# HuiGuanLab/Lite-MKD

Measured on AMD Instinct MI355X. Metric: episodes/sec (5-way 5-shot, 8x224^2 frames), higher is better.
Workload: dtype f32

## Files before the change

include/lmkd.h:

```cpp
#ifndef LMKD_H
#define LMKD_H
#ifdef __cplusplus
extern "C" {
#endif

int lmkd_abi_version(void);
const char* lmkd_last_error(void);
int lmkd_device_check(int device);
int lmkd_set_activation_dtype(int mode);
int lmkd_get_activation_dtype(void);

int lmkd_gemm_f32(char layA, char layB, int M, int N, int K, float alpha, const float* A, long lda, long sA,
                  const float* B, long ldb, long sB, float beta, float* C, long ldc, long sC, const float* bias,
                  int relu, int batch, void* stream);
int lmkd_gemm_set_mode(int mode);
int lmkd_gemm_set_tile(int t);
long lmkd_gemm_ticket_words(void);
int lmkd_gemm_f32_splitk(char layA, char layB, int M, int N, int K, float alpha, const float* A, long lda, long sA,
                         const float* B, long ldb, long sB, float beta, float* C, long ldc, long sC, const float* bias,
                         int relu, int batch, void* workspace, long ws_bytes, unsigned* tickets, void* stream);

long lmkd_conv2d_packed_weight_elems(int Cout, int Cin, int Cs, int KH, int KW, int mode);
int lmkd_conv2d_pack_weights(const float* w_oihw, float* wp, int Cout, int Cin, int Cs, int KH, int KW, int mode ,
                             void* stream);
int lmkd_conv2d_fwd_row_tiles(int N, int H, int W, int Cout, int KH, int KW, int stride, int pad);
int lmkd_conv2d_fwd_row_tiles_cs(int N, int H, int W, int Cs, int Cout, int KH, int KW, int stride, int pad);
int lmkd_set_elementwise_wg_per_cu(int n);
int lmkd_conv_set_compute_dtype(int mode);
typedef struct lmkd_amax_desc {
  const void* x_words;
  const void* dy_words;
  void* out_words;
  const void* ref_words;
  int flags;
} lmkd_amax_desc;
#define LMKD_AMAX_FENCED 1
int lmkd_h2_fence_eval(const void* const* words, void* const* refs, int n, int* flags, void* stream);
long lmkd_conv_h2_fallbacks(void);
int lmkd_amax(const float* x, long n, void* word, void* stream);
long lmkd_amax_words(void);
long lmkd_conv2d_plane_elems(int ncols, int Kp);
long lmkd_conv_h2_launches(void);
int lmkd_conv2d_repack_multi(const float* const* ws, void* const* wfs, const int* dims, int n, void* stream);
int lmkd_conv2d_split_weights(const float* wp, void* wf, int ncols, int Kp, void* stream);
int lmkd_conv_get_compute_dtype(void);
int lmkd_conv_set_wgrad_planes(int on);
int lmkd_conv_set_patch(int on);
int lmkd_conv_set_stem_patch(int on);
int lmkd_conv_set_s2_patch(int on);
int lmkd_conv_set_wgrad_win16(int on);
int lmkd_conv_set_wgrad_stem(int on);
int lmkd_conv_set_wgrad_window(int on);
int lmkd_conv_set_patch16(int on);
int lmkd_conv_set_persistent(int on);
int lmkd_conv_set_xcd_mode(int mode);
int lmkd_conv_set_tile(int id);
int lmkd_conv2d_fwd(const float* x, const float* wp_fwd, float* y, float* stat_partial, int N, int H, int W, int Cs, int Cout,
                    int KH, int KW, int stride, int pad, void* stream);
int lmkd_conv2d_fwd_pre(const float* x_raw, const float* pre_stats, const float* wp_fwd, float* y, float* stat_partial, int N, int H,
                        int W, int Cs, int Cout, int KH, int KW, int stride, int pad, void* stream);
int lmkd_conv2d_fwd_bn(const float* x, const float* wp_fwd, float* y, const float* bn_stats, const float* res , int relu,
                       int N, int H, int W, int Cs, int Cout, int KH, int KW, int stride, int pad, void* stream,
                       const lmkd_amax_desc* amax );
int lmkd_conv2d_bwd_data(const float* dy, const float* wp_dgrad, float* dx, int N, int H, int W, int Cin, int Cout, int KH, int KW,
                         int stride, int pad, int accumulate, void* stream);
int lmkd_conv2d_bwd_data_bn_tiles(int N, int H, int W, int Cin, int Cout, int KH, int KW, int stride, int pad);
int lmkd_conv2d_bwd_data_bn(const float* dy, const float* wp_dgrad, float* dx, const float* bn_x, const float* bn_stats, float* part,
                            int N, int H, int W, int Cin, int Cout, int KH, int KW, int stride, int pad, void* stream);
long lmkd_conv2d_bwd_weight_workspace(int N, int H, int W, int Cs, int Cout, int KH, int KW, int stride, int pad);
int lmkd_conv2d_bwd_weight(const float* x, const float* dy, float* dw_oihw, float* workspace, long ws_bytes, int N, int H, int W,
                           int Cs, int Cin, int Cout, int KH, int KW, int stride, int pad, void* stream);
int lmkd_conv2d_bwd_weight_pre(const float* x_raw, const float* pre_stats, const float* dy, float* dw_oihw, float* workspace,
                               long ws_bytes, int N, int H, int W, int Cs, int Cin, int Cout, int KH, int KW, int stride, int pad,
                               void* stream);

int lmkd_conv2d_plan(int kind, int N, int H, int W, int Cs, int Cin, int Cout, int KH, int KW, int stride, int pad, int* info_host);

int lmkd_conv2d_bwd_weight_acc(const float* x, const float* pre_stats, const float* dy, float* dw_oihw, float* workspace, long ws_bytes,
                               int N, int H, int W, int Cs, int Cin, int Cout, int KH, int KW, int stride, int pad, void* stream);

int lmkd_frames_u8_to_nhwc4(const unsigned char* src, float* dst, const int* crop_y, const int* crop_x, const int* flip, int F, int Hs,
                            int Ws, int H, int W, int frames_per_video, void* stream);
int lmkd_resize_plan(int in_size, int out_size, int* bounds_host, int* coeffs_host);
int lmkd_resize_pass_u8(const unsigned char* src, unsigned char* dst, const int* bounds_dev, const int* coeffs_dev, int ksize, long outer,
                        int n_in, int n_out, long inner, void* stream);
int lmkd_frames_resize_crop_nhwc4(const unsigned char* src, float* dst, const int* bounds_h, const int* coeffs_h, int ksize_h,
                                  const int* bounds_v, const int* coeffs_v, int ksize_v, const int* crop_y, const int* crop_x,
                                  const int* flip, int F, int Hs, int Ws, int Hr, int Wr, int H, int W, int frames_per_video, void* stream);
int lmkd_nchw3_to_nhwc4(const float* x_nchw, float* y_nhwc4, int N, int H, int W, void* stream, void* amax_words);
long lmkd_ticket_words(void);
int lmkd_bn_finalize(const float* partial, int T, int C, long count, const float* gamma, const float* beta, float* running_mean,
                     float* running_var, float momentum, float eps, float* stats, double* scratch, unsigned* tickets, void* stream,
                     const lmkd_amax_desc* amax );
int lmkd_bn_running_update(float* running_mean, float* running_var, const float* stats, int C, float momentum, void* stream);
int lmkd_bn_running_update_multi(float* const* running_mean, float* const* running_var, const float* const* stats_first,
                                 const float* const* stats_second, const int* C, int n, float momentum, void* stream);
int lmkd_bn_running_update_multi_nbt(float* const* running_mean, float* const* running_var, const float* const* stats_first,
                                     const float* const* stats_second, long long* const* num_batches_tracked, const int* C, int n,
                                     float momentum, void* stream);
int lmkd_bn_eval_stats(int C, const float* gamma, const float* beta, const float* running_mean, const float* running_var, float eps,
                       float* stats, void* stream);
int lmkd_bn_apply(const float* x, const float* stats, const float* res, const float* rstats, float* y, long rows, int C, int relu,
                  int res_mode, unsigned* mask_bits, void* stream);
long lmkd_bn_bwd_workspace(int C);
int lmkd_bn_backward(const float* dy, const float* x, const float* yact, const float* stats, const float* gamma, float* dx,
                     float* g_out, float* dgamma, float* dbeta, float* coef, void* workspace, unsigned* tickets, long rows, int C,
                     int mask_mode, int accumulate_param_grads, void* stream);
int lmkd_bn_backward_part(const float* part, int T, const float* dy, const float* x, const float* stats, const float* gamma, float* dx,
                          float* dgamma, float* dbeta, float* coef, void* workspace, unsigned* tickets, long rows, int C,
                          int accumulate_param_grads, void* stream);
int lmkd_relu_backward(const float* dy, const float* y, float* g, long n, void* stream);
int lmkd_bn_relu_maxpool_fwd(const float* x, const float* stats, float* y, unsigned char* idx, float* cmax, int N, int H, int W, int C,
                             void* stream);
int lmkd_maxpool_bwd(const float* dy, const unsigned char* idx, float* g, int N, int H, int W, int C, void* stream);
int lmkd_bn_backward_stats(const float* dy, const float* cmax, const float* stats, const float* gamma, float* dgamma, float* dbeta,
                           float* coef, void* workspace, unsigned* tickets, long pooled_rows, long count, int C, int accumulate_param_grads,
                           void* stream);
int lmkd_stem_unpool_bn_bwd(const float* dy, const unsigned char* idx, const float* c, const float* stats, const float* coef, float* dc,
                            int N, int H, int W, int C, void* stream, const lmkd_amax_desc* amax );
int lmkd_adaptive_maxpool_mean_fwd(const float* x, float* y, int F, int H, int W, int C, void* stream);
int lmkd_adaptive_maxpool_mean_bwd(const float* x, const float* dy, float* dx, int F, int H, int W, int C, void* stream);
long lmkd_colsum_workspace(int C);
int lmkd_colsum(const float* a, const float* b, float* out, long rows, int C, int accumulate, void* workspace, unsigned* tickets,
                void* stream);

int lmkd_dropout_mask(float* mask, long n, float p, unsigned long long seed, void* stream);
int lmkd_dropout_mask_dev(float* mask, long n, float p, const unsigned long long* seed_dev, void* stream);
int lmkd_add_pe(const float* x, const float* pe, const float* mask, float* y, long rows, int D, int L, void* stream);
int lmkd_mul(const float* a, const float* b, float* out, long n, void* stream);
int lmkd_axpby(const float* x, float* y, float alpha, float beta, long n, void* stream);
int lmkd_trx_tuple_ln_fwd(const float* P, const float* bk, const float* bv, const float* gamma, const float* beta, const int* rowmap,
                          float* Kn, float* Khat, float* V, float* rstd, int NV, int L, int D, float eps, void* stream);
int lmkd_layernorm_bwd_rows(float* dK_inout, const float* Khat, const float* rstd, const float* gamma, long rows, int D, void* stream);
int lmkd_trx_tuple_bwd_gather(const float* dKraw, const float* dV, const int* rowmap, float* dP, int NV, int L, int D, void* stream);
int lmkd_segment_softmax_fwd(float* S, long rows, long ld, int nseg, const int* seg_off, const int* seg_cnt, void* stream);
int lmkd_segment_softmax_bwd(const float* P, float* dP_inout, long rows, long ld, int nseg, const int* seg_off, const int* seg_cnt,
                             void* stream);
// ... 68 lines not shown
```

lite-mkd_amd/_lib.py:

```python
import ctypes
import os
import re

from . import _audit

_HERE = os.path.dirname(os.path.abspath(__file__))
_ROOT = os.path.dirname(_HERE)
HEADER = os.path.join(_ROOT, "include", "lmkd.h")
LIB_PATH = os.environ.get("LMKD_LIB") or os.path.join(_HERE, "liblmkd_hip.so")

_CT = {
    "int": ctypes.c_int, "long": ctypes.c_long, "float": ctypes.c_float, "char": ctypes.c_char,
    "long long": ctypes.c_longlong, "unsigned long long": ctypes.c_ulonglong,
}


def parse_header(path=HEADER):
    txt = open(path).read()
    txt = re.sub(r"/\*.*?\*/", " ", txt, flags=re.S)
    protos = {}
    for m in re.finditer(r"\b(int|long|const char\s*\*)\s+(lmkd_\w+)\s*\(([^)]*)\)\s*;", txt):
        ret, name, args = m.group(1), m.group(2), m.group(3).strip()
        restype = ctypes.c_char_p if "char" in ret else _CT[ret]
        argtypes = []
        if args and args != "void":
            for a in args.split(","):
                a = a.strip()
                if "*" in a:
                    argtypes.append(ctypes.c_void_p)
                else:
                    toks = a.replace("const ", "").split()
                    ty = " ".join(toks[:-1])
                    argtypes.append(_CT[ty])
        protos[name] = (restype, argtypes)
    return protos


class _Lib:
    def __init__(self):
        if not os.path.exists(LIB_PATH):
            raise RuntimeError(
                "liblmkd_hip.so not found at %s: build it with `python lite-mkd_amd/build.py` "
                "(there is no CPU or PyTorch fallback for the hot path)" % LIB_PATH)
        import torch
        self.cdll = ctypes.CDLL(LIB_PATH)
        self.protos = parse_header()
        for name, (restype, argtypes) in self.protos.items():
            fn = getattr(self.cdll, name)
            fn.restype = restype
            fn.argtypes = argtypes
        if os.environ.get("LMKD_PATCH16"):
            self.cdll.lmkd_conv_set_patch16(int(os.environ["LMKD_PATCH16"]))
        if os.environ.get("LMKD_WGRAD_WINDOW"):
            self.cdll.lmkd_conv_set_wgrad_window(int(os.environ["LMKD_WGRAD_WINDOW"]))
        if os.environ.get("LMKD_CONV_PERSISTENT", "1") == "0":
            self.cdll.lmkd_conv_set_persistent(0)

    def last_error(self):
        return self.cdll.lmkd_last_error().decode()

    def call(self, name, *args):
        if _audit.ON:
            _audit.check(name)
        rc = getattr(self.cdll, name)(*args)
        if rc != 0:
            raise RuntimeError("%s failed (%d): %s" % (name, rc, self.last_error()))

    def value(self, name, *args):
        return getattr(self.cdll, name)(*args)


_lib = None


def lib():
    global _lib
    if _lib is None:
        _lib = _Lib()
    return _lib
```

lite-mkd_amd/csrc/conv.hip:

```cpp
#include "gemm_core.h"
#include <atomic>
#include <mutex>

struct ConvGemmArgs {
  const float* src;
  const float* wpk;
  float* out;
  float* stat_partial;
  int N, Hs, Ws, Cs;
  int Hr, Wr, rows_per_class, tiles_per_class;
  int sh;
  int Ho, Wo, Co, omul;
  int Kp, cps, nclass;
  int n_rt, n_ct, xcd_mode;
  int taps_pm1;
  int grid_step;
  int grid_total;
  int same;
  int halo;
  int accum;
  const float* ep_stats;
  const float* ep_res;
  int ep_relu;
  const float* pre_stats;
// ... 784 lines not shown
template <class Cfg, bool SMALLC, int STATS, bool BF16 = false>
static void launch_conv_cfg(ConvGemmArgs a, int ncols, hipStream_t s) {
  conv_set_tiles(a, Cfg::BM);
  a.n_ct = cdiv(ncols, Cfg::BN);
  a.xcd_mode = (a.n_ct >= 8 && (a.n_ct & 7) == 0) ? 1 : 0;
  if (g_xcd_mode == 0) a.xcd_mode = 0;
  const dim3 grid(xcd_grid(a.n_rt, a.n_ct, a.xcd_mode));
  if constexpr (STATS == 1 && !SMALLC && !BF16) {
    if (a.pre_stats) {
      hipLaunchKernelGGL((conv_gemm_kernel<Cfg, SMALLC, STATS, BF16, true>), grid, dim3(Cfg::THREADS), 0, s, a);
      return;
    }
  }
  hipLaunchKernelGGL((conv_gemm_kernel<Cfg, SMALLC, STATS, BF16>), grid, dim3(Cfg::THREADS), 0, s, a);
}

static inline void lmkd_lds_attr_once(std::atomic<unsigned long long>& mask, const void* fn, int bytes) {
  int d = 0;
  if (hipGetDevice(&d) != hipSuccess) d = 0;
  const unsigned long long bit = 1ull << (d & 63);
  if (mask.load(std::memory_order_acquire) & bit) return;
  const hipError_t err = hipFuncSetAttribute(fn, hipFuncAttributeMaxDynamicSharedMemorySize, bytes);
  if (err != hipSuccess) {
    lmkd_set_error("hipFuncSetAttribute(MaxDynamicSharedMemorySize = %d): %s", bytes, hipGetErrorString(err));
    return;
  }
  mask.fetch_or(bit, std::memory_order_release);
}

struct PersistOcc { std::atomic<int> n{0}; int lds[8]; int occ[8]; std::mutex mu; };
static int lmkd_cu_count() {
  static std::atomic<int> n{0};
  int v = n.load(std::memory_order_relaxed);
  if (v) return v;
  int d = 0;
  hipDeviceProp_t pr;
  if (hipGetDevice(&d) != hipSuccess || hipGetDeviceProperties(&pr, d) != hipSuccess || pr.multiProcessorCount < 1) return 256;
  n.store(pr.multiProcessorCount, std::memory_order_relaxed);
  return pr.multiProcessorCount;
}
static int g_conv_persist = 1;
extern "C" int lmkd_conv_set_persistent(int on) { g_conv_persist = on ? 1 : 0; return LMKD_OK; }
template <class K>
static int persistent_grid(PersistOcc& c, K kernel, int threads, size_t lds, int total) {
  if (!g_conv_persist) return total;
  int occ = 0;
  {
    std::lock_guard<std::mutex> lk(c.mu);
    const int n = c.n.load();
    for (int i = 0; i < n; ++i) if (c.lds[i] == (int)lds) occ = c.occ[i];
    if (!occ) {
      if (hipOccupancyMaxActiveBlocksPerMultiprocessor(&occ, kernel, threads, lds) != hipSuccess || occ < 1) occ = 1;
      if (n < 8) { c.lds[n] = (int)lds; c.occ[n] = occ; c.n.store(n + 1); }
    }
  }
  const int slots = occ * lmkd_cu_count();
  if (total <= slots) return total;
  const int rounds = cdiv(total, slots);
  const int g = (cdiv(total, rounds) + 7) & ~7;
  return g < total ? g : total;
}

static int patch_halo(const ConvGemmArgs& a) {
  if (!g_conv_patch || !(g_conv_x3 || g_conv_bf16) || a.Cs % 32 != 0 || a.sh != 1) return -1;
  const bool plain = a.nclass == 1 && a.Hs == a.Ho && a.Ws == a.Wo;
  const bool classes = a.nclass == 4 && a.Hr == a.Hs && a.Wr == a.Ws;
  if (!plain && !classes) return -1;
  int halo = 0;
  for (int c = 0; c < a.nclass; ++c)
    for (int t = 0; t < a.ntap[c]; ++t) {
      const int sft = a.taps[c][t].dh * a.Ws + a.taps[c][t].dw;
      halo = std::max(halo, sft < 0 ? -sft : sft);
    }
  return halo <= PATCH_HALO_MAX ? halo : -1;
}
static inline bool conv_same_size(int H, int W, int KH, int KW, int stride, int pad) {
  return g_conv_patch && stride == 1 && conv_out(H, KH, stride, pad) == H && conv_out(W, KW, stride, pad) == W && (KH / 2) * W + KW / 2 <= PATCH_HALO_MAX;
}

static int g_conv_s2_patch = 1;
extern "C" int lmkd_conv_set_s2_patch(int on) { g_conv_s2_patch = on ? 1 : 0; return LMKD_OK; }
static int g_patch16 = 1;
extern "C" int lmkd_conv_set_patch16(int on) { g_patch16 = on < 0 ? 0 : (on > 2 ? 2 : on); return LMKD_OK; }

#ifdef LMKD_STAMPS
extern "C" int lmkd_debug_stamps(unsigned long long* host, int zero) {
  if (zero) {
    void* p = nullptr;
    if (hipGetSymbolAddress(&p, HIP_SYMBOL(g_lmkd_stamps)) != hipSuccess) return LMKD_EHIP;
    return hipMemset(p, 0, sizeof(g_lmkd_stamps)) == hipSuccess ? LMKD_OK : LMKD_EHIP;
  }
  return hipMemcpyFromSymbol(host, HIP_SYMBOL(g_lmkd_stamps), sizeof(g_lmkd_stamps)) == hipSuccess ? LMKD_OK : LMKD_EHIP;
}
#endif
static inline int taps_within_one(const ConvGemmArgs& a) {
  for (int c = 0; c < a.nclass; ++c)
    for (int t = 0; t < a.ntap[c]; ++t)
      if (a.taps[c][t].dh < -1 || a.taps[c][t].dh > 1 || a.taps[c][t].dw < -1 || a.taps[c][t].dw > 1) return 0;
  return 1;
}
template <class Cfg>
static void launch_conv_patch(ConvGemmArgs a, int ncols, int halo, hipStream_t s) {
  conv_set_tiles(a, Cfg::BM);
  a.taps_pm1 = taps_within_one(a);
  a.n_ct = cdiv(ncols, Cfg::BN);
  a.xcd_mode = (a.n_ct >= 8 && (a.n_ct & 7) == 0) ? 1 : 0;
  if (g_xcd_mode == 0) a.xcd_mode = 0;
  const dim3 grid(xcd_grid(a.n_rt, a.n_ct, a.xcd_mode));
  a.halo = halo;
  const int npl = (g_conv_bf16 || g_lmkd_act_bf16) ? 1 : 3;
  size_t lds = patch_lds_bytes(Cfg::BM, halo, npl);
#define LMKD_PATCH(NPROD, PRE, IO)                                                                                             \
  do {                                                                                                                         \
    static std::atomic<unsigned long long> attr_done{0};                                                                       \
    static PersistOcc pocc;                                                                                                    \
    lmkd_lds_attr_once(attr_done, reinterpret_cast<const void*>(&conv_patch_x3_kernel<Cfg, NPROD, PRE, IO>),                   \
                       (int)patch_lds_bytes(Cfg::BM, PATCH_HALO_MAX, NPROD == 1 ? 1 : 3));                                     \
    a.grid_total = (int)grid.x;                                                                                                \
    const dim3 pgrid(NPROD == 3 ? persistent_grid(pocc, conv_patch_x3_kernel<Cfg, NPROD, PRE, IO>, Cfg::THREADS, lds, a.grid_total) : a.grid_total); \
    a.grid_step = (int)pgrid.x;                                                                                                \
    hipLaunchKernelGGL((conv_patch_x3_kernel<Cfg, NPROD, PRE, IO>), pgrid, dim3(Cfg::THREADS), lds, s, a);                     \
  } while (0)
  if constexpr (Cfg::THREADS == 256 && Cfg::BM == 128) {
    const bool h2_on_32 = g_patch16 == 1 && Cfg::BN == 64 && a.Co <= 64 && g_conv_h2 && a.h2_xw && !a.src2 && !a.ep_stats;
    if (g_patch16 && g_conv_x3 && !g_lmkd_act_bf16 && !h2_on_32) {
#define LMKD_PATCH16(NPROD, PRE, EP)                                                                                           \
  do {                                                                                                                         \
    t_amax_recorded = true;                                                                                                    \
    static std::atomic<unsigned long long> attr_done{0};                                                                       \
    lmkd_lds_attr_once(attr_done, reinterpret_cast<const void*>(&conv_patch16_x3_kernel<Cfg, NPROD, PRE, EP>),                 \
                       (int)patch_lds_bytes(Cfg::BM, PATCH_HALO_MAX, 3));                                                      \
    hipLaunchKernelGGL((conv_patch16_x3_kernel<Cfg, NPROD, PRE, EP>), grid, dim3(Cfg::THREADS), lds, s, a);                    \
  } while (0)
      if (a.src2) {
#define LMKD_PATCH16S(NPROD, EP)                                                                                               \
  do {                                                                                                                         \
    t_amax_recorded = true;                                                                                                    \
    static std::atomic<unsigned long long> attr_done{0};                                                                       \
    lmkd_lds_attr_once(attr_done, reinterpret_cast<const void*>(&conv_patch16_x3_kernel<Cfg, NPROD, false, EP, true>),         \
                       (int)patch_lds_bytes(Cfg::BM, PATCH_HALO_MAX, 3));                                                      \
    hipLaunchKernelGGL((conv_patch16_x3_kernel<Cfg, NPROD, false, EP, true>), grid, dim3(Cfg::THREADS), lds, s, a);            \
  } while (0)
        if (a.ep_stats) {
          if (g_conv_x3 == 9) LMKD_PATCH16S(9, true);
          else if (g_conv_h2 && a.h2_xw) { LMKD_PATCH16S(3, true); ++g_h2_launches; }
          else LMKD_PATCH16S(6, true);
        }
        else if (g_conv_h2 && a.h2_xw) { LMKD_PATCH16S(3, false); ++g_h2_launches; }
        else { if (g_conv_x3 == 9) LMKD_PATCH16S(9, false); else LMKD_PATCH16S(6, false); }
#undef LMKD_PATCH16S
        return;
      }
      if (a.ep_stats) {
        if (g_conv_x3 == 9) LMKD_PATCH16(9, false, true);
        else if (g_conv_h2 && a.h2_xw) { LMKD_PATCH16(3, false, true); ++g_h2_launches; }
        else LMKD_PATCH16(6, false, true);
      }
      else if (a.pre_stats) {
        if (g_conv_x3 == 9) LMKD_PATCH16(9, true, false);
        else if (g_conv_h2 && a.h2_xw) { LMKD_PATCH16(3, true, false); ++g_h2_launches; }
        else LMKD_PATCH16(6, true, false);
      }
      else if (a.bnb_x) {
#define LMKD_PATCH16B(NPROD)                                                                                                   \
  do {                                                                                                                         \
    t_amax_recorded = true;                                                                                                    \
    static std::atomic<unsigned long long> attr_done{0};                                                                       \
    lmkd_lds_attr_once(attr_done, reinterpret_cast<const void*>(&conv_patch16_x3_kernel<Cfg, NPROD, false, false, false, true>), \
                       (int)patch_lds_bytes(Cfg::BM, PATCH_HALO_MAX, 3));                                                      \
    hipLaunchKernelGGL((conv_patch16_x3_kernel<Cfg, NPROD, false, false, false, true>), grid, dim3(Cfg::THREADS), lds, s, a);  \
  } while (0)
        if (g_conv_h2 && a.h2_xw) { LMKD_PATCH16B(3); ++g_h2_launches; }
        else if (g_conv_x3 == 9) LMKD_PATCH16B(9);
        else LMKD_PATCH16B(6);
#undef LMKD_PATCH16B
      }
      else if (g_conv_h2 && a.h2_xw) { LMKD_PATCH16(3, false, false); ++g_h2_launches; }
      else { if (g_conv_x3 == 9) LMKD_PATCH16(9, false, false); else LMKD_PATCH16(6, false, false); }
#undef LMKD_PATCH16
      return;
    }
  }
  if (g_conv_h2 && a.h2_xw && !a.ep_stats && !g_lmkd_act_bf16) {
    t_amax_recorded = true;
    lds = patch_lds_bytes(Cfg::BM, halo, 2);
    if (a.pre_stats) LMKD_PATCH(3, true, 0); else LMKD_PATCH(3, false, 0);
    ++g_h2_launches;
    return;
  }
  if (a.ep_stats) {
    if (g_conv_bf16) LMKD_PATCH(1, false, 4);
    else if (g_conv_x3 == 9) LMKD_PATCH(9, false, 4);
    else LMKD_PATCH(6, false, 4);
  } else if (g_lmkd_act_bf16) LMKD_PATCH(1, false, 3);
  else if (a.pre_stats) {
    if (g_conv_bf16) LMKD_PATCH(1, true, 0);
    else if (g_conv_x3 == 9) LMKD_PATCH(9, true, 0);
    else LMKD_PATCH(6, true, 0);
  } else {
    if (g_conv_bf16) LMKD_PATCH(1, false, 0);
    else if (g_conv_x3 == 9) LMKD_PATCH(9, false, 0);
    else LMKD_PATCH(6, false, 0);
  }
#undef LMKD_PATCH
}

template <class Cfg>
static void launch_conv_patch_1p(ConvGemmArgs a, int ncols, int halo, hipStream_t s) {
  conv_set_tiles(a, Cfg::BM);
  a.taps_pm1 = taps_within_one(a);
  a.n_ct = cdiv(ncols, Cfg::BN);
  a.xcd_mode = (a.n_ct >= 8 && (a.n_ct & 7) == 0) ? 1 : 0;
  if (g_xcd_mode == 0) a.xcd_mode = 0;
  const dim3 grid(xcd_grid(a.n_rt, a.n_ct, a.xcd_mode));
  a.halo = halo;
  const size_t lds = patch_lds_bytes(Cfg::BM, halo, 1);
#define LMKD_PATCH1(PRE, IO)                                                                                                   \
  do {                                                                                                                         \
    static std::atomic<unsigned long long> attr_done{0};                                                                       \
    lmkd_lds_attr_once(attr_done, reinterpret_cast<const void*>(&conv_patch_x3_kernel<Cfg, 1, PRE, IO>),                       \
                       (int)patch_lds_bytes(Cfg::BM, PATCH_HALO_MAX, 1));                                                      \
    a.grid_total = (int)grid.x;                                                                                                \
    const dim3 pgrid(a.grid_total);                  \
    a.grid_step = (int)pgrid.x;                                                                                                \
    hipLaunchKernelGGL((conv_patch_x3_kernel<Cfg, 1, PRE, IO>), pgrid, dim3(Cfg::THREADS), lds, s, a);                         \
  } while (0)
  if (a.ep_stats) LMKD_PATCH1(false, 4);
  else if (g_lmkd_act_bf16) LMKD_PATCH1(false, 3);
  else if (a.pre_stats) LMKD_PATCH1(true, 0);
  else LMKD_PATCH1(false, 0);
#undef LMKD_PATCH1
}

template <class Cfg, bool SMALLC, bool STATS>
static void launch_conv_x3(ConvGemmArgs a, int ncols, hipStream_t s) {
  conv_set_tiles(a, Cfg::BM);
  a.n_ct = cdiv(ncols, Cfg::BN);
  a.xcd_mode = (a.n_ct >= 8 && (a.n_ct & 7) == 0) ? 1 : 0;
  if (g_xcd_mode == 0) a.xcd_mode = 0;
  const dim3 grid(xcd_grid(a.n_rt, a.n_ct, a.xcd_mode));
  (void)STATS;
  if constexpr (!SMALLC) {
    if (a.ep_stats) {
      if (g_conv_bf16) hipLaunchKernelGGL((conv_gemm_x3_kernel<Cfg, false, true, 1, false, 4>), grid, dim3(Cfg::THREADS), 0, s, a);
      else if (g_conv_x3 == 9) hipLaunchKernelGGL((conv_gemm_x3_kernel<Cfg, false, true, 9, false, 4>), grid, dim3(Cfg::THREADS), 0, s, a);
      else hipLaunchKernelGGL((conv_gemm_x3_kernel<Cfg, false, true, 6, false, 4>), grid, dim3(Cfg::THREADS), 0, s, a);
      return;
    }
  }
  if (g_lmkd_act_bf16) {
    if constexpr (SMALLC) hipLaunchKernelGGL((conv_gemm_x3_kernel<Cfg, true, true, 1, false, 2>), grid, dim3(Cfg::THREADS), 0, s, a);
    else hipLaunchKernelGGL((conv_gemm_x3_kernel<Cfg, false, true, 1, false, 3>), grid, dim3(Cfg::THREADS), 0, s, a);
    return;
  }
  if constexpr (!SMALLC) {
    if (a.pre_stats) {
      if (g_conv_bf16) hipLaunchKernelGGL((conv_gemm_x3_kernel<Cfg, false, true, 1, true>), grid, dim3(Cfg::THREADS), 0, s, a);
      else if (g_conv_x3 == 9) hipLaunchKernelGGL((conv_gemm_x3_kernel<Cfg, false, true, 9, true>), grid, dim3(Cfg::THREADS), 0, s, a);
      else hipLaunchKernelGGL((conv_gemm_x3_kernel<Cfg, false, true, 6, true>), grid, dim3(Cfg::THREADS), 0, s, a);
      return;
    }
  }
  if (g_conv_bf16) hipLaunchKernelGGL((conv_gemm_x3_kernel<Cfg, SMALLC, true, 1>), grid, dim3(Cfg::THREADS), 0, s, a);
  else if (g_conv_x3 == 9) hipLaunchKernelGGL((conv_gemm_x3_kernel<Cfg, SMALLC, true, 9>), grid, dim3(Cfg::THREADS), 0, s, a);
  else hipLaunchKernelGGL((conv_gemm_x3_kernel<Cfg, SMALLC, true, 6>), grid, dim3(Cfg::THREADS), 0, s, a);
}

template <bool SMALLC, int STATS>
// ... 720 lines not shown
```

lite-mkd_amd/csrc/conv_patch.h:

```cpp
#pragma once

#define PATCH_HALO_MAX 57

template <int NPL> struct PatchRow { static constexpr int BYTES = NPL == 1 ? 80 : (NPL == 2 ? 144 : 208); };

static inline size_t patch_lds_bytes(int bm, int halo, int npl) { return (size_t)(bm + 2 * halo + 1) * (npl == 1 ? 80 : (npl == 2 ? 144 : 208)); }

#ifdef LMKD_STAMPS
__device__ unsigned long long g_lmkd_stamps[4096 * 8];
#define STAMP(k) do { if (threadIdx.x == 0 && (blockIdx.x & 63) == 0 && (blockIdx.x >> 6) < 4096) g_lmkd_stamps[(blockIdx.x >> 6) * 8 + (k)] = __builtin_amdgcn_s_memtime(); } while (0)
#else
#define STAMP(k) do { } while (0)
#endif


template <class Cfg>
__device__ __forceinline__ void patch_h2_epilogue(const ConvGemmArgs& a, f32x16 (&acc)[Cfg::TM][Cfg::TN], const int* s_out, float* s_red, int rt,
                                                  int n0, int wm, int wn, int lane, int tid, int seg, int row0, int M, float h2_ix, float h2_iw) {
  const int cl0 = wn * (Cfg::TN * 32) + (lane & 31);
  const bool bnb = a.bnb_x != nullptr;
  float s1[Cfg::TN], s2[Cfg::TN];
  float amo = 0.f;
  const bool plain = a.nclass == 1;
  const int rows = M - row0 < Cfg::BM ? M - row0 : Cfg::BM;
// ... 411 lines not shown
      read_a(0);
      if (AHEAD) read_a(1);
      __builtin_amdgcn_sched_barrier(0);
#pragma unroll
      for (int g = 0; g < 2; ++g) {
        const int ga = AHEAD ? g : 0;
        if (!AHEAD && g == 1) {
          __builtin_amdgcn_sched_barrier(0);
          read_a(1);
          __builtin_amdgcn_sched_barrier(0);
        }
#pragma unroll
        for (int j = 0; j < Cfg::TN; ++j) {
          if constexpr (NPROD == 1) {
            const bf16x8 b0 = x3_as_bf16(rb[j * 2 + g]);
#pragma unroll
            for (int i = 0; i < Cfg::TM; ++i) acc[i][j] = __builtin_amdgcn_mfma_f32_32x32x16_bf16(av[ga][0][i], b0, acc[i][j], 0, 0, 0);
          } else if constexpr (NPROD == 3) {
            const f16x8 b0 = __builtin_bit_cast(f16x8, rb[j * 4 + g * 2 + 0]), b1 = __builtin_bit_cast(f16x8, rb[j * 4 + g * 2 + 1]);
#pragma unroll
            for (int i = 0; i < Cfg::TM; ++i) {
              f32x16 c = acc[i][j];
              c = __builtin_amdgcn_mfma_f32_32x32x16_f16(__builtin_bit_cast(f16x8, av[ga][0][i]), b1, c, 0, 0, 0);
              c = __builtin_amdgcn_mfma_f32_32x32x16_f16(__builtin_bit_cast(f16x8, av[ga][1][i]), b0, c, 0, 0, 0);
              c = __builtin_amdgcn_mfma_f32_32x32x16_f16(__builtin_bit_cast(f16x8, av[ga][0][i]), b0, c, 0, 0, 0);
              acc[i][j] = c;
            }
          } else {
            const bf16x8 b0 = x3_as_bf16(rb[j * 6 + g * 3 + 0]), b1 = x3_as_bf16(rb[j * 6 + g * 3 + 1]), b2 = x3_as_bf16(rb[j * 6 + g * 3 + 2]);
#pragma unroll
            for (int i = 0; i < Cfg::TM; ++i) {
              f32x16 c = acc[i][j];
              if (NPROD == 9) {
                c = __builtin_amdgcn_mfma_f32_32x32x16_bf16(av[ga][2][i], b2, c, 0, 0, 0);
                c = __builtin_amdgcn_mfma_f32_32x32x16_bf16(av[ga][1][i], b2, c, 0, 0, 0);
                c = __builtin_amdgcn_mfma_f32_32x32x16_bf16(av[ga][2][i], b1, c, 0, 0, 0);
              }
              c = __builtin_amdgcn_mfma_f32_32x32x16_bf16(av[ga][1][i], b1, c, 0, 0, 0);
              c = __builtin_amdgcn_mfma_f32_32x32x16_bf16(av[ga][0][i], b2, c, 0, 0, 0);
              c = __builtin_amdgcn_mfma_f32_32x32x16_bf16(av[ga][2][i], b0, c, 0, 0, 0);
              c = __builtin_amdgcn_mfma_f32_32x32x16_bf16(av[ga][0][i], b1, c, 0, 0, 0);
              c = __builtin_amdgcn_mfma_f32_32x32x16_bf16(av[ga][1][i], b0, c, 0, 0, 0);
              c = __builtin_amdgcn_mfma_f32_32x32x16_bf16(av[ga][0][i], b0, c, 0, 0, 0);
              acc[i][j] = c;
            }
          }
        }
      }
      if (++k_tp == ntap) { k_tp = 0; ++k_cc; }
      __builtin_amdgcn_sched_barrier(0);
      x3_landed(rbn);
      x3_landed(rp);
      __builtin_amdgcn_sched_barrier(0);
      if (t + 2 < nk) issue_b(rb);
    };
    PSTAMP(1);
    if (nk > 0) {
      x3_landed(rp);
      x3_landed(rb0);
      x3_landed(rb1);
      __builtin_amdgcn_sched_barrier(0);
      PSTAMP(2);
      int t = 0;
      for (; t + 1 < nk; t += 2) {
        step(t, rb0, rb1, avp0, avp1);
        step(t + 1, rb1, rb0, avp1, avp0);
      }
      if (t < nk) step(t, rb0, rb1, avp0, avp1);
    }
    PSTAMP(3);
    if constexpr (NPROD == 3) {
      patch_h2_epilogue<Cfg>(a, acc, s_out, s_red, cur.rt, n0, wm, wn, lane, tid, cur.seg, row0, M, h2_ix, h2_iw);
    } else {
      x3_epilogue<Cfg, true, OUT16, EP>(a, acc, s_out, s_red, cur.rt, n0, wm, wn, lane, tid, neg);
    }
    PSTAMP(4);
    if (!PERSIST || Ln < 0) break;
    if (!inv) __syncthreads();
    cur = nxt;
    Lc = Ln;
    ++it;
  }
}
```

Before: 51.32.

## Add ring-buffered persistent patch kernel for 64-channel 3x3 split-half conv

Adds a persistent conv kernel for the 64-channel 3x3 stride-1 two-plane (h2) case. It keeps a rolling LDS ring of input pixel rows so consecutive output tiles handled by one block reuse the overlapping halo instead of reloading it, and it prefetches the next tile's new rows while the current tile's MFMAs run. The aim is to cut redundant global loads and halo staging per tile. In exchange it adds a specialised code path with strict eligibility conditions, more LDS use, and a fixed row-ordering assumption about ring slots.

```diff
diff --git a/include/lmkd.h b/include/lmkd.h
--- a/include/lmkd.h
+++ b/include/lmkd.h
@@ -53,6 +53,7 @@
 int lmkd_conv_set_wgrad_window(int on);
 int lmkd_conv_set_patch16(int on);
 int lmkd_conv_set_persistent(int on);
+int lmkd_conv_set_patch_ring(int on);
 int lmkd_conv_set_xcd_mode(int mode);
 int lmkd_conv_set_tile(int id);
 int lmkd_conv2d_fwd(const float* x, const float* wp_fwd, float* y, float* stat_partial, int N, int H, int W, int Cs, int Cout,
diff --git a/lite-mkd_amd/_lib.py b/lite-mkd_amd/_lib.py
--- a/lite-mkd_amd/_lib.py
+++ b/lite-mkd_amd/_lib.py
@@ -55,6 +55,8 @@
             self.cdll.lmkd_conv_set_wgrad_window(int(os.environ["LMKD_WGRAD_WINDOW"]))
         if os.environ.get("LMKD_CONV_PERSISTENT", "1") == "0":
             self.cdll.lmkd_conv_set_persistent(0)
+        if os.environ.get("LMKD_CONV_PATCH_RING", "1") == "0":
+            self.cdll.lmkd_conv_set_patch_ring(0)
 
     def last_error(self):
         return self.cdll.lmkd_last_error().decode()
diff --git a/lite-mkd_amd/csrc/conv.hip b/lite-mkd_amd/csrc/conv.hip
--- a/lite-mkd_amd/csrc/conv.hip
+++ b/lite-mkd_amd/csrc/conv.hip
@@ -890,6 +890,12 @@
 extern "C" int lmkd_conv_set_s2_patch(int on) { g_conv_s2_patch = on ? 1 : 0; return LMKD_OK; }
 static int g_patch16 = 1;
 extern "C" int lmkd_conv_set_patch16(int on) { g_patch16 = on < 0 ? 0 : (on > 2 ? 2 : on); return LMKD_OK; }
+static int g_patch_ring = 1;
+extern "C" int lmkd_conv_set_patch_ring(int on) { g_patch_ring = on ? 1 : 0; return LMKD_OK; }
+static inline bool patch_ring_fits(const ConvGemmArgs& a, int halo) {
+  return g_patch_ring && g_conv_persist && a.nclass == 1 && a.n_ct == 1 && !a.src2 && a.Cs == 64 && a.cps == 2 && a.ntap[0] == 9 && a.taps_pm1 &&
+         halo <= 64 && a.n_rt > 0;
+}
 
 #ifdef LMKD_STAMPS
 extern "C" int lmkd_debug_stamps(unsigned long long* host, int zero) {
@@ -992,6 +998,24 @@
   if (g_conv_h2 && a.h2_xw && !a.ep_stats && !g_lmkd_act_bf16) {
     t_amax_recorded = true;
     lds = patch_lds_bytes(Cfg::BM, halo, 2);
+    if constexpr (Cfg::BM == 128 && Cfg::BN == 64 && Cfg::THREADS == 256 && Cfg::TN == 1) {
+      if (patch_ring_fits(a, halo)) {
+        const size_t rlds = patch_ring_lds_bytes();
+#define LMKD_PATCH_RING(PRE)                                                                                                   \
+  do {                                                                                                                         \
+    static std::atomic<unsigned long long> attr_done{0};                                                                       \
+    static PersistOcc pocc;                                                                                                    \
+    lmkd_lds_attr_once(attr_done, reinterpret_cast<const void*>(&conv_patch_ring_kernel<Cfg, PRE>), (int)rlds);               \
+    a.grid_total = a.n_rt;                                                                                                     \
+    a.grid_step = persistent_grid(pocc, conv_patch_ring_kernel<Cfg, PRE>, Cfg::THREADS, rlds, a.n_rt);                         \
+    hipLaunchKernelGGL((conv_patch_ring_kernel<Cfg, PRE>), dim3(a.grid_step), dim3(Cfg::THREADS), rlds, s, a);                 \
+  } while (0)
+        if (a.pre_stats) LMKD_PATCH_RING(true); else LMKD_PATCH_RING(false);
+#undef LMKD_PATCH_RING
+        ++g_h2_launches;
+        return;
+      }
+    }
     if (a.pre_stats) LMKD_PATCH(3, true, 0); else LMKD_PATCH(3, false, 0);
     ++g_h2_launches;
     return;
diff --git a/lite-mkd_amd/csrc/conv_patch.h b/lite-mkd_amd/csrc/conv_patch.h
--- a/lite-mkd_amd/csrc/conv_patch.h
+++ b/lite-mkd_amd/csrc/conv_patch.h
@@ -517,3 +517,208 @@
     ++it;
   }
 }
+
+#define RING_ROWB 272
+#define RING_ROWS 256
+static inline size_t patch_ring_lds_bytes() { return (size_t)(RING_ROWS + 1) * RING_ROWB; }
+
+template <class Cfg, bool PRE>
+__global__ __launch_bounds__(Cfg::THREADS, 2) void conv_patch_ring_kernel(ConvGemmArgs) {
+  static_assert(Cfg::BM == 128 && Cfg::THREADS == 256 && Cfg::BN == 64 && Cfg::TN == 1, "layer 1's two-plane tile");
+  __shared__ ConvGemmArgs s_args;
+  {
+    const unsigned* ksrc = (const unsigned*)__builtin_amdgcn_kernarg_segment_ptr();
+    unsigned* kdst = reinterpret_cast<unsigned*>(&s_args);
+    for (int i = threadIdx.x; i < (int)(sizeof(ConvGemmArgs) / 4); i += Cfg::THREADS) kdst[i] = ksrc[i];
+  }
+  __syncthreads();
+  ConvGemmArgs a;
+  {
+    constexpr int NW = (int)(offsetof(ConvGemmArgs, ntap) / 4);
+    unsigned* aw = reinterpret_cast<unsigned*>(&a);
+    const unsigned* lw = reinterpret_cast<const unsigned*>(&s_args);
+#pragma unroll
+    for (int i = 0; i < NW; ++i) aw[i] = __builtin_amdgcn_readfirstlane(lw[i]);
+  }
+  constexpr int ROWB = RING_ROWB, NTAP = 9, NK = 2 * NTAP;
+  constexpr int LPR = 16, RPP = Cfg::THREADS / LPR, NI = Cfg::BM / RPP;
+  using LB = X3FragB<Cfg::TN, 2>;
+  extern __shared__ __attribute__((aligned(16))) unsigned char psm[];
+  __shared__ unsigned short s_mask_lut[64];
+  __shared__ float s_red[Cfg::WM * Cfg::BN * 2];
+  const int tid = threadIdx.x;
+  const int lane = tid & 63, wave = tid >> 6;
+  const int wm = wave / Cfg::WN, wn = wave % Cfg::WN;
+  const int h = lane >> 5;
+  const int a_row = wm * (Cfg::TM * 32) + (lane & 31);
+  const unsigned zero_addr = (unsigned)(RING_ROWS * ROWB + 16 * h);
+  const __amdgpu_buffer_rsrc_t prs = x3_rsrc(a.src, (long)a.N * a.Hs * a.Ws * a.Cs * 4);
+  const int pk = (tid & (LPR - 1)) * 4;
+  const long src_pixels = (long)a.N * a.Hs * a.Ws;
+  const int G = a.grid_step, T = a.n_rt, b = (int)blockIdx.x;
+  const int r = (G & 7) == 0 ? (b & 7) * (G >> 3) + (b >> 3) : b;
+  const int t_beg = (int)((long)r * T / G), t_end = (int)((long)(r + 1) * T / G);
+  if (t_beg >= t_end) return;
+  const Tap my_tap = s_args.taps[0][lane < NTAP ? lane : 0];
+  int sh_px[NTAP], kofs[NTAP];
+#pragma unroll
+  for (int tp = 0; tp < NTAP; ++tp) {
+    sh_px[tp] = __builtin_amdgcn_readlane(my_tap.dh * a.Ws + my_tap.dw, tp);
+    kofs[tp] = __builtin_amdgcn_readlane(my_tap.kofs, tp);
+  }
+  if (tid < 64) {
+    const int rb = tid & 7, cb = tid >> 3;
+    unsigned m = 0;
+    for (int tp = 0; tp < NTAP; ++tp) {
+      const int dh = s_args.taps[0][tp].dh, dw = s_args.taps[0][tp].dw;
+      if (((rb >> (dh + 1)) & 1) && ((cb >> (dw + 1)) & 1)) m |= 1u << tp;
+    }
+    s_mask_lut[tid] = (unsigned short)m;
+  }
+  for (int j = tid; j < ROWB / 4; j += Cfg::THREADS) reinterpret_cast<unsigned*>(psm + RING_ROWS * ROWB)[j] = 0u;
+  const unsigned h2_wbits = *reinterpret_cast<const unsigned*>(reinterpret_cast<const unsigned short*>(a.wpk) + (long)a.Co * a.Kp * 16);
+  LB lb;
+  lb.init(reinterpret_cast<const unsigned short*>(a.wpk) + (long)a.Co * a.Kp * 16 + 32, a.Co, a.Kp, wn * (Cfg::TN * 32), lane, false);
+  __syncthreads();
+  const float h2_iw = 1.f / h2_scale(h2_wbits);
+
+  u32x4 rp[NI];
+  unsigned r_ok = 0u;
+  int r_q0 = 0;
+  float4 psc = float4(), psh = float4();
+  auto issue_rows = [&](int q0, int seg) {
+    const long pix0 = (long)q0 + tid / LPR;
+    r_q0 = q0;
+    r_ok = 0u;
+#pragma unroll
+    for (int i = 0; i < NI; ++i) {
+      const long pix = pix0 + RPP * i;
+      const bool ok = pix >= 0 && pix < src_pixels;
+      r_ok |= ok ? 1u << i : 0u;
+      rp[i] = __builtin_amdgcn_raw_buffer_load_b128(prs, ok ? (unsigned)((pix * a.Cs + pk) * 4) : X3_OOB, 0, 0);
+    }
+    if (PRE) {
+      const float* pre_tab = a.pre_stats + (long)seg * 5 * a.Cs;
+      psc = *reinterpret_cast<const float4*>(pre_tab + 2 * a.Cs + pk);
+      psh = *reinterpret_cast<const float4*>(pre_tab + 3 * a.Cs + pk);
+    }
+  };
+  auto store_rows = [&](float h2_sx) {
+#pragma unroll
+    for (int i = 0; i < NI; ++i) {
+      const unsigned slot = (unsigned)(r_q0 + tid / LPR + RPP * i) & (RING_ROWS - 1);
+      unsigned char* d = psm + slot * ROWB + pk * 2;
+      float4 v = make_float4(__uint_as_float(rp[i].x), __uint_as_float(rp[i].y), __uint_as_float(rp[i].z), __uint_as_float(rp[i].w));
+      if (PRE && ((r_ok >> i) & 1u)) {
+        v.x = fmaxf(fmaf(v.x, psc.x, psh.x), 0.f); v.y = fmaxf(fmaf(v.y, psc.y, psh.y), 0.f);
+        v.z = fmaxf(fmaf(v.z, psc.z, psh.z), 0.f); v.w = fmaxf(fmaf(v.w, psc.w, psh.w), 0.f);
+      }
+      uint2 q0, q1;
+      h2_split4(v, h2_sx, q0, q1);
+      *reinterpret_cast<uint2*>(d) = q0;
+      *reinterpret_cast<uint2*>(d + 128) = q1;
+    }
+  };
+
+  bool ring_ok = false;
+  int it = 0;
+  for (int tile = t_beg; tile < t_end; ++tile, ++it) {
+    PSTAMP(0);
+    const SegTile sg = seg_tile(a, tile, Cfg::BM);
+    const int row0 = sg.row0, M = sg.mend;
+    const bool has_next = tile + 1 < t_end;
+    const SegTile sn = seg_tile(a, has_next ? tile + 1 : tile, Cfg::BM);
+    const bool next_on = has_next && sn.seg == sg.seg && sn.row0 == row0 + Cfg::BM;
+    const unsigned h2_xbits = a.h2_xw[sg.seg * LMKD_AMAX_SEG_WORDS + (tid & (LMKD_AMAX_SLOTS - 1)) * LMKD_AMAX_STRIDE];
+    u32x4 rb[2][LB::NR];
+    lb.load(kofs[0], rb[0]);
+    lb.load(kofs[1], rb[1]);
+    unsigned a_pix[Cfg::TM], a_mask[Cfg::TM];
+#pragma unroll
+    for (int i = 0; i < Cfg::TM; ++i) {
+      const int m = row0 + a_row + 32 * i;
+      a_pix[i] = (unsigned)m;
+      a_mask[i] = 0u;
+      if (m < M) {
+        const int n = fdiv(m, a.div_hw);
+        const int rem = m - n * a.Hs * a.Ws;
+        const int hh = fdiv(rem, a.div_w), ww = rem - hh * a.Ws;
+        const unsigned Hs = (unsigned)a.Hs, Ws = (unsigned)a.Ws;
+        const unsigned rbits = ((unsigned)(hh - 1) < Hs ? 1u : 0u) | ((unsigned)hh < Hs ? 2u : 0u) | ((unsigned)(hh + 1) < Hs ? 4u : 0u);
+        const unsigned cbits = ((unsigned)(ww - 1) < Ws ? 1u : 0u) | ((unsigned)ww < Ws ? 2u : 0u) | ((unsigned)(ww + 1) < Ws ? 4u : 0u);
+        a_mask[i] = s_mask_lut[rbits | (cbits << 3)];
+      }
+    }
+    unsigned v = h2_xbits;
+#pragma unroll
+    for (int o = 32; o >= 1; o >>= 1) {
+      const unsigned u = (unsigned)__shfl_xor((int)v, o, 64);
+      v = u > v ? u : v;
+    }
+    const float h2_sx = h2_scale(__builtin_amdgcn_readfirstlane(v));
+    const float h2_ix = 1.f / h2_sx;
+    PSTAMP(1);
+    if (!ring_ok) {
+      issue_rows(row0 - 64, sg.seg);
+      store_rows(h2_sx);
+      issue_rows(row0 + 64, sg.seg);
+    }
+    store_rows(h2_sx);
+    __syncthreads();
+    if (next_on) issue_rows(sn.row0 + 64, sn.seg);
+    ring_ok = next_on;
+    unsigned at[Cfg::TM][NTAP];
+#pragma unroll
+    for (int tp = 0; tp < NTAP; ++tp)
+#pragma unroll
+      for (int i = 0; i < Cfg::TM; ++i)
+        at[i][tp] = ((a_mask[i] >> tp) & 1u) ? ((a_pix[i] + (unsigned)sh_px[tp]) & (RING_ROWS - 1)) * ROWB + 16 * h : zero_addr;
+    f32x16 acc[Cfg::TM][Cfg::TN];
+#pragma unroll
+    for (int i = 0; i < Cfg::TM; ++i)
+#pragma unroll
+      for (int j = 0; j < Cfg::TN; ++j)
+#pragma unroll
+        for (int e = 0; e < 16; ++e) acc[i][j][e] = 0.f;
+    bf16x8 av[2][2][2][Cfg::TM];
+    auto read_a = [&](int t, bf16x8 (&dst)[2][2][Cfg::TM]) {
+      const int tp = t % NTAP, cc = t / NTAP;
+#pragma unroll
+      for (int g = 0; g < 2; ++g)
+#pragma unroll
+        for (int p = 0; p < 2; ++p)
+#pragma unroll
+          for (int i = 0; i < Cfg::TM; ++i) dst[g][p][i] = *reinterpret_cast<const bf16x8*>(psm + at[i][tp] + p * 128 + cc * 64 + g * 32);
+    };
+    x3_landed(rb[0]);
+    x3_landed(rb[1]);
+    read_a(0, av[0]);
+    __builtin_amdgcn_sched_barrier(0);
+    PSTAMP(2);
+#pragma unroll
+    for (int t = 0; t < NK; ++t) {
+      if (t + 1 < NK) read_a(t + 1, av[(t + 1) & 1]);
+#pragma unroll
+      for (int g = 0; g < 2; ++g)
+#pragma unroll
+        for (int j = 0; j < Cfg::TN; ++j) {
+          const f16x8 b0 = __builtin_bit_cast(f16x8, rb[t & 1][j * 4 + g * 2 + 0]), b1 = __builtin_bit_cast(f16x8, rb[t & 1][j * 4 + g * 2 + 1]);
+#pragma unroll
+          for (int i = 0; i < Cfg::TM; ++i) {
+            f32x16 c = acc[i][j];
+            c = __builtin_amdgcn_mfma_f32_32x32x16_f16(__builtin_bit_cast(f16x8, av[t & 1][g][0][i]), b1, c, 0, 0, 0);
+            c = __builtin_amdgcn_mfma_f32_32x32x16_f16(__builtin_bit_cast(f16x8, av[t & 1][g][1][i]), b0, c, 0, 0, 0);
+            c = __builtin_amdgcn_mfma_f32_32x32x16_f16(__builtin_bit_cast(f16x8, av[t & 1][g][0][i]), b0, c, 0, 0, 0);
+            acc[i][j] = c;
+          }
+        }
+      __builtin_amdgcn_sched_barrier(0);
+      if (t + 1 < NK) x3_landed(rb[(t + 1) & 1]);
+      __builtin_amdgcn_sched_barrier(0);
+      if (t + 2 < NK) lb.load(kofs[(t + 2) % NTAP] + ((t + 2) / NTAP) * LMKD_BK, rb[t & 1]);
+    }
+    PSTAMP(3);
+    patch_h2_epilogue<Cfg>(a, acc, nullptr, s_red, tile, 0, wm, wn, lane, tid, sg.seg, row0, M, h2_ix, h2_iw);
+    PSTAMP(4);
+  }
+}
```

Result: no change. 51.48 (median of 6 runs) (+0.3%).
